# snap-research/3dgp

Measured on AMD Instinct MI355X. Metric: generator-forward img/s @256^2, 64 steps, higher is better.
Workload: dtype f32; 1 GPU; BASELINE configs[2]: ImageNet 256x256, 64(+64) ray steps, cmax 512, c_dim 1000, tri-plane 512^2 x 96, full HIP path; batch_per_gpu=16, global_batch=16, img_resolution=256, num_ray_steps=64, depth_adaptor=False, parallelism=dp1 (batch-sharded, weights replicated)

## Files before the change

3dgp_amd/csrc/sampling.hip:

```cpp
#include "common.h"

namespace {

constexpr int MAXS = 256;
constexpr int RAYS_PER_BLOCK = 4;
constexpr int MAXS_PASS = 512;
constexpr int MAXS_LONG = 1024;

template <int MS>
struct alignas(16) WaveScratchT {
    float z[MS];
    float sig[MS];
    float w[MS + 4];
    float cdf[MS];
    float bins[MS];
    float col[3][MS];
};
using WaveScratch = WaveScratchT<MAXS>;

template <int MS> struct alignas(16) MarchScratchT { float z[MS]; float sig[MS]; float w[MS + 4]; };
template <> struct alignas(16) MarchScratchT<MAXS> : WaveScratch {};
template <int MS> struct alignas(16) UnifyScratchT { float z[MS]; };
template <> struct alignas(16) UnifyScratchT<MAXS> : WaveScratch {};

__device__ __forceinline__ void wave_sync() {
    __builtin_amdgcn_fence(__ATOMIC_ACQ_REL, "wavefront");
    __builtin_amdgcn_wave_barrier();
}

__device__ __forceinline__ float s2t(float s, float t_near, float t_far) { return s * t_far + (1.0f - s) * t_near; }

template <bool LONGX>
__device__ __forceinline__ float exp_neg(float x) { return LONGX ? (float)exp(-(double)x) : expf(-x); }

#define TDGP_CLASSICAL_ALPHA(LONGX, z, sig, i, S, flags, cut_thr, alpha, fac)                                        \
    do {                                                                                                            \
        alpha = 0.f; fac = 1.0f;                                                                                    \
        if ((i) < (S)) {                                                                                            \
            const float delta = ((i) < (S) - 1) ? (z[(i) + 1] - z[i]) : (((flags) & 1) ? 1e10f : 1e-3f);            \
            float sp = ((flags) & 8) ? (sig[i] > 0.f ? sig[i] : 0.f) : softplus20f(sig[i]);                         \
            if (sp < cut_thr) sp = 0.f;              \
            alpha = 1.0f - exp_neg<LONGX>(delta * sp);                                                              \
            fac = (1.0f - alpha) + 1e-10f;                                                                          \
        }                                                                                                           \
    } while (0)

#define TDGP_MIP_ALPHA(LONGX, z, sig, i, S, M, density_bias, cut_thr, alpha, fac)                                    \
    do {                                                                                                            \
        alpha = 0.f; fac = 1.0f;                                                                                    \
        if ((i) < (M)) {                                                                                            \
            float delta, smid;                                                                                      \
            if ((i) < (S) - 1) { delta = z[(i) + 1] - z[i]; smid = (sig[i] + sig[(i) + 1]) / 2.f; }                 \
            else { delta = 1e10f; smid = sig[(S) - 1]; }                                                            \
            float sp = softplus20f(smid + density_bias);                                                            \
            if (sp < cut_thr) sp = 0.f;                                                \
            float dd = sp * delta;                                                                                  \
            alpha = 1.0f - exp_neg<LONGX>(dd);                                                                      \
            fac = (1.0f - alpha) + 1e-10f;                                                                          \
        }                                                                                                           \
    } while (0)

#define TDGP_MARCH_PASS(wi, incl64, alpha, fac, carry)                   \
    const double incl64 = wave_scan_f64<true>((double)(fac)) * (carry);  \
    const float incl = (float)incl64;                                    \
    const float excl = wave_shr1_f32(incl, (float)(carry));              \
    const float wi = (alpha) * excl;
#define TDGP_MARCH_PASS2(wi0, wi1, i1, alpha, fac)                                                                          \
    const double s0 = wave_scan_f64<true>((double)fac[0]), s1 = wave_scan_f64<true>((double)fac[1]);                        \
    const double c1 = wave_last_f64(s0);                                                                                    \
    const double i1 = s1 * c1;                                                                                              \
    const float incl0 = (float)s0, incl1 = (float)i1;                                                                       \
    const float wi0 = alpha[0] * wave_shr1_f32(incl0, 1.0f), wi1 = alpha[1] * wave_shr1_f32(incl1, (float)c1);

template <bool LONGX = false>
__device__ void march_classical_lds(const float* z, const float* sig, float* w, int S, int flags, float cut_thr, float& final_T, float& wagg) {
    const int l = lane_id();
    double carry = 1.0;
    float wsum = 0.0f;
    if (S > 64 && S <= 128) {
        float alpha[2], fac[2];
#pragma unroll
        for (int c = 0; c < 2; c++) {
            const int i = 64 * c + l;
            TDGP_CLASSICAL_ALPHA(LONGX, z, sig, i, S, flags, cut_thr, alpha[c], fac[c]);
        }
        TDGP_MARCH_PASS2(wi0, wi1, i1, alpha, fac)
        w[l] = wi0; wsum += wi0;
        if (64 + l < S) { w[64 + l] = wi1; wsum += wi1; }
        carry = wave_last_f64(i1);
    } else
    for (int base = 0; base < S; base += 64) {
        const int i = base + l;
        float alpha, fac;
        TDGP_CLASSICAL_ALPHA(LONGX, z, sig, i, S, flags, cut_thr, alpha, fac);
        TDGP_MARCH_PASS(wi, incl64, alpha, fac, carry)
        if (i < S) { w[i] = wi; wsum += wi; }
        carry = wave_last_f64(incl64);
    }
    wagg = wave_sum_f32(wsum);
    final_T = (float)carry;
    wave_sync();
    if ((flags & 2) && l == 0) w[S - 1] += (1.0f - wagg);
    wave_sync();
}

template <bool LONGX = false>
__device__ void march_mip_lds(const float* z, const float* sig, float* w, int S, int flags, float density_bias, float cut_thr, float& final_T,
                              float& wagg) {
    const int l = lane_id();
    const int M = (flags & 1) ? S : S - 1;
    double carry = 1.0;
    float wsum = 0.0f;
    for (int base = 0; base < M; base += 64) {
        const int i = base + l;
        float alpha, fac;
        TDGP_MIP_ALPHA(LONGX, z, sig, i, S, M, density_bias, cut_thr, alpha, fac);
        TDGP_MARCH_PASS(wi, incl64, alpha, fac, carry)
        if (i < M) { w[i] = wi; wsum += wi; }
        carry = wave_last_f64(incl64);
    }
    wagg = wave_sum_f32(wsum);
    final_T = (float)carry;
    wave_sync();
}

__device__ float torch_order_sum_lds(const float* w1, int n, float eps) {
    const int l = lane_id();
    if (n >= 8) {
        const int nv = n >> 3, nilp = nv >> 2;
        const int col = l & 7, a = (l >> 3) & 3;
        float acc = 0.f;
        for (int i = 0; i < nilp; i++) acc = __fadd_rn(acc, __fadd_rn(w1[(4 * i + a) * 8 + col], eps));
        for (int j = 4 * nilp; j < nv; j++) {
            const float v = __fadd_rn(w1[j * 8 + col], eps);
            if (a == 0) acc = __fadd_rn(acc, v);
        }
        float p = __shfl(acc, col, 64);
        p = __fadd_rn(p, __shfl(acc, col + 8, 64));
        p = __fadd_rn(p, __shfl(acc, col + 16, 64));
        p = __fadd_rn(p, __shfl(acc, col + 24, 64));
        float fin = 0.f;
        for (int k = nv * 8; k < n; k++) fin = __fadd_rn(fin, __fadd_rn(w1[k], eps));
#pragma unroll
        for (int c = 0; c < 8; c++) fin = __fadd_rn(fin, __int_as_float(__builtin_amdgcn_readlane(__float_as_int(p), c)));
        return fin;
    }
    float acc[4] = {0.f, 0.f, 0.f, 0.f};
    const int nilp = n >> 2;
    if (nilp)
        for (int k = 0; k < 4; k++) acc[k] = __fadd_rn(acc[k], __fadd_rn(w1[k], eps));
    for (int r = 4 * nilp; r < n; r++) acc[0] = __fadd_rn(acc[0], __fadd_rn(w1[r], eps));
    for (int k = 1; k < 4; k++) acc[0] = __fadd_rn(acc[0], acc[k]);
    return acc[0];
}

__device__ __forceinline__ float torch_order_sum_62(const float* w1, int n, float eps) {
    const int l = lane_id();
    const int col = l & 7, a = (l >> 3) & 3;
    float acc = 0.f;
    acc = __fadd_rn(acc, __fadd_rn(w1[a * 8 + col], eps));
#pragma unroll
    for (int j = 4; j < 7; j++) {
        const float v = __fadd_rn(w1[j * 8 + col], eps);
        if (a == 0) acc = __fadd_rn(acc, v);
    }
    float p = __shfl(acc, col, 64);
    p = __fadd_rn(p, __shfl(acc, col + 8, 64));
    p = __fadd_rn(p, __shfl(acc, col + 16, 64));
    p = __fadd_rn(p, __shfl(acc, col + 24, 64));
    float fin = 0.f;
#pragma unroll
    for (int k = 56; k < 62; k++) {
        const float t = __fadd_rn(fin, __fadd_rn(w1[k], eps));
        fin = k < n ? t : fin;
    }
#pragma unroll
    for (int c = 0; c < 8; c++) fin = __fadd_rn(fin, __int_as_float(__builtin_amdgcn_readlane(__float_as_int(p), c)));
    return fin;
}

template <int NV>
__device__ __forceinline__ void smooth_read(const float* w, int Wn, float (&nv)[NV]) {
    const int l = lane_id();
#pragma unroll
    for (int c = 0; c < NV; c++) {
        const int i = l + 64 * c;
        if (i < Wn) {
            float a = (i - 1 >= 0) ? w[i - 1] : -INFINITY, b = w[i], d = (i + 1 < Wn) ? w[i + 1] : -INFINITY;
            float t0 = a > b ? a : b;
            float t1 = b > d ? b : d;
            nv[c] = (t0 + t1) / 2.f + 0.01f;
        }
    }
}
template <int NV>
__device__ __forceinline__ void smooth_write(float* w, int Wn, const float (&nv)[NV]) {
    const int l = lane_id();
#pragma unroll
    for (int c = 0; c < NV; c++) {
        const int i = l + 64 * c;
        if (i < Wn) w[i] = nv[c];
    }
}
__device__ __forceinline__ void offset_weights(float* w, int Wn) {
    for (int i = lane_id(); i < Wn; i += 64) w[i] = w[i] + 1e-5f;
}
template <bool ROW62>
__device__ __forceinline__ void pdf_cdf(const float* z, const float* w, float* bins, float* cdf, int S, int Wn) {
    const int l = lane_id();
    const float eps = 1e-5f;
    const int nb = S - 1, ns = Wn - 2;
    for (int i = l; i < nb; i += 64) bins[i] = 0.5f * (z[i] + z[i + 1]);
    const float totf = ROW62 ? torch_order_sum_62(w + 1, ns, eps) : torch_order_sum_lds(w + 1, ns, eps);
    double carry = 0.0;
    if (l == 0) cdf[0] = 0.f;
    for (int base = 0; base < ns; base += 64) {
        const int i = base + l;
        float pdf = (i < ns) ? (w[1 + i] + eps) / totf : 0.f;
        double incl = wave_scan_f64<false>((double)pdf) + carry;
        if (i < ns) cdf[i + 1] = (float)incl;
        carry = wave_last_f64(incl);
    }
}
__device__ __forceinline__ int cdf_search(const float* cdf, int nc, float uu) {
    int lo = 0, hi = nc;
    while (lo < hi) {
        int mid = (lo + hi) >> 1;
        if (cdf[mid] <= uu) lo = mid + 1; else hi = mid;
    }
    return lo;
}
__device__ __forceinline__ float cdf_sample(const float* cdf, const float* bins, int nb, int ns, int ind, float uu, int& below, int& above) {
    const float eps = 1e-5f;
    below = ind - 1 < 0 ? 0 : ind - 1;
    above = ind > ns ? ns : ind;
    const float cb = cdf[below], ca = cdf[above];
    const float bb = bins[below < nb ? below : nb - 1], ba = bins[above < nb ? above : nb - 1];
    float denom = ca - cb;
    if (denom < eps) denom = 1.f;
    return bb + (uu - cb) / denom * (ba - bb);
}

template <typename SC, typename GetU, typename Emit>
__device__ void importance_lds(SC& sc, int S, int Wn, GetU getu, int N, int mip, Emit emit) {
    const int l = lane_id();
    float* w = sc.w;
    constexpr int CAP = sizeof(sc.z) / sizeof(float), NV = (CAP > MAXS ? CAP : MAXS) / 64;
    if (mip) {
        float nv[NV];
        smooth_read<NV>(w, Wn, nv);
        wave_sync();
        smooth_write<NV>(w, Wn, nv);
    } else {
        offset_weights(w, Wn);
    }
    wave_sync();
    const int nb = S - 1, ns = Wn - 2, nc = ns + 1;
    pdf_cdf<false>(sc.z, w, sc.bins, sc.cdf, S, Wn);
    wave_sync();
    for (int j = l; j < N; j += 64) {
        const float uu = getu(j);
        const int ind = cdf_search(sc.cdf, nc, uu);
        int below, above;
        const float smp = cdf_sample(sc.cdf, sc.bins, nb, ns, ind, uu, below, above);
        emit(j, smp, ind, below, above);
    }
}

__device__ __forceinline__ float strat_one(float u, int k, int S, float step, int marcher) {
    auto lin = [&](int q) { return (S == 1) ? 0.f : ((q < S / 2) ? __fmaf_rn(step, (float)q, 0.f) : __fmaf_rn(-step, (float)(S - 1 - q), 1.f)); };
    if (marcher == 0) {
        const float lower = (k == 0) ? lin(0) : 0.5f * (lin(k) + lin(k - 1));
        const float upper = (k == S - 1) ? lin(S - 1) : 0.5f * (lin(k + 1) + lin(k));
        return lower + (upper - lower) * u;
    }
    const float delta = (float)((1.0 - 0.0) / (double)(S - 1));
    return lin(k) + u * delta;
}

__global__ __launch_bounds__(256) void stratified_kernel(const float* __restrict__ u, float* __restrict__ sdist, float* __restrict__ tdist,
                                                        int64_t n, int S, int marcher, float t_near, float t_far) {
    const float step = (1.f - 0.f) / (float)(S - 1);
    for (int64_t i = blockIdx.x * (int64_t)blockDim.x + threadIdx.x; i < n; i += (int64_t)gridDim.x * blockDim.x) {
        const float s = strat_one(u[i], (int)(i % S), S, step, marcher);
        sdist[i] = s;
        if (tdist) tdist[i] = s2t(s, t_near, t_far);
    }
}

__global__ __launch_bounds__(256) void stratified4_kernel(const float4* __restrict__ u, float4* __restrict__ sdist, float4* __restrict__ tdist,
                                                         int64_t n4, int S, int marcher, float t_near, float t_far) {
    const float step = (1.f - 0.f) / (float)(S - 1);
    const int S4 = S >> 2;
    for (int64_t i = blockIdx.x * (int64_t)blockDim.x + threadIdx.x; i < n4; i += (int64_t)gridDim.x * blockDim.x) {
        const int k = (int)(i % S4) * 4;
        const float4 uu = u[i];
        const float4 s = make_float4(strat_one(uu.x, k, S, step, marcher), strat_one(uu.y, k + 1, S, step, marcher), strat_one(uu.z, k + 2, S, step, marcher),
                                     strat_one(uu.w, k + 3, S, step, marcher));
        sdist[i] = s;
        if (tdist) tdist[i] = make_float4(s2t(s.x, t_near, t_far), s2t(s.y, t_near, t_far), s2t(s.z, t_near, t_far), s2t(s.w, t_near, t_far));
    }
}

__global__ __launch_bounds__(256) void density_activation_kernel(const float* __restrict__ x, float* __restrict__ y, int64_t n, int relu, float bias) {
    for (int64_t i = blockIdx.x * (int64_t)blockDim.x + threadIdx.x; i < n; i += (int64_t)gridDim.x * blockDim.x)
        y[i] = relu ? (x[i] > 0.f ? x[i] : 0.f) : softplus20f(x[i] + bias);
}

template <int MS>
__global__ __launch_bounds__(256) void ray_march_kernel(const float* __restrict__ colors, const float* __restrict__ dens,
                                                       const float* __restrict__ depths, float* __restrict__ rgb, float* __restrict__ depth_o,
                                                       float* __restrict__ weights, float* __restrict__ final_T, int64_t rays, int S, int C,
                                                       int marcher, int flags, float density_bias, float cut_thr) {
    __shared__ MarchScratchT<MS> scratch[RAYS_PER_BLOCK];
    const int wv = threadIdx.x >> 6, l = lane_id();
    const int64_t r = (int64_t)blockIdx.x * RAYS_PER_BLOCK + wv;
    if (r >= rays) return;
    MarchScratchT<MS>& sc = scratch[wv];
    for (int i = l; i < S; i += 64) { sc.z[i] = depths[r * S + i]; sc.sig[i] = dens[r * S + i]; }
    wave_sync();
    float fT, wagg;
    const int M = (marcher == 0) ? S : ((flags & 1) ? S : S - 1);
    if (MS > MAXS && S > MAXS) {
        if (marcher == 0) march_classical_lds<(MS > MAXS)>(sc.z, sc.sig, sc.w, S, flags, cut_thr, fT, wagg);
        else march_mip_lds<(MS > MAXS)>(sc.z, sc.sig, sc.w, S, flags, density_bias, cut_thr, fT, wagg);
    } else
    if (marcher == 0) march_classical_lds(sc.z, sc.sig, sc.w, S, flags, cut_thr, fT, wagg);
    else march_mip_lds(sc.z, sc.sig, sc.w, S, flags, density_bias, cut_thr, fT, wagg);
    if (weights) for (int i = l; i < M; i += 64) weights[r * M + i] = sc.w[i];
    for (int c = 0; c <= C; c++) {
        float acc = 0.0f;
        for (int i = l; i < M; i += 64) {
            float v;
            if (c < C) {
                v = colors[(r * S + i) * C + c];
                if (marcher == 1 && i < S - 1) v = (v + colors[(r * S + i + 1) * C + c]) / 2.f;
            } else {
                v = sc.z[i];
                if (marcher == 1 && i < S - 1) v = (v + sc.z[i + 1]) / 2.f;
            }
            acc += sc.w[i] * v;
        }
        float out = wave_sum_f32(acc);
        if (marcher == 1 && c < C) {
            if (flags & 4) out = out + 1.0f - wagg;
            out = out * 2.0f - 1.0f;
        }
        if (l == 0) { if (c < C) rgb[r * C + c] = out; else depth_o[r] = out; }
    }
    if (l == 0) final_T[r] = fT;
}

template <int MS>
__global__ __launch_bounds__(256) void sample_importance_kernel(const float* __restrict__ z, const float* __restrict__ weights,
                                                               const float* __restrict__ u, float* __restrict__ samples, int32_t* __restrict__ inds,
                                                               int32_t* __restrict__ below, int32_t* __restrict__ above, float* __restrict__ cdf_o,
                                                               int64_t rays, int S, int Wn, int N, int mip) {
    __shared__ WaveScratchT<MS> scratch[RAYS_PER_BLOCK];
    const int wv = threadIdx.x >> 6, l = lane_id();
    const int64_t r = (int64_t)blockIdx.x * RAYS_PER_BLOCK + wv;
    if (r >= rays) return;
    WaveScratchT<MS>& sc = scratch[wv];
    for (int i = l; i < S; i += 64) sc.z[i] = z[r * S + i];
    for (int i = l; i < Wn; i += 64) sc.w[i] = weights[r * Wn + i];
    wave_sync();
    importance_lds(sc, S, Wn, [&](int j) { return u[r * N + j]; }, N, mip, [&](int j, float smp, int ind, int bl, int ab) {
        samples[r * N + j] = smp;
        if (inds) { inds[r * N + j] = ind; below[r * N + j] = bl; above[r * N + j] = ab; }
    });
    if (cdf_o) for (int i = l; i < Wn - 1; i += 64) cdf_o[r * (Wn - 1) + i] = sc.cdf[i];
}

template <int NS>
__device__ __forceinline__ void stable_ranks_n(const float* key, int M, int* rank) {
    const int l = lane_id();
    float k[NS];
#pragma unroll
    for (int c = 0; c < NS; c++) { const int i = l + 64 * c; k[c] = i < M ? key[i] : 0.f; rank[c] = 0; }
#pragma unroll 4
    for (int m = 0; m < M; m++) {
        const float km = key[m];
#pragma unroll
        for (int c = 0; c < NS; c++) {
            const int i = l + 64 * c;
            rank[c] += (km < k[c] || (km == k[c] && m < i)) ? 1 : 0;
        }
    }
}
template <int NR>
__device__ __forceinline__ void stable_ranks(const float* key, int M, int (&rank)[NR]) {
    static_assert(NR == MAXS / 64 || NR == MAXS_PASS / 64 || NR == MAXS_LONG / 64, "stable_ranks: 4, 8 or 16 slots");
#pragma unroll
    for (int c = 0; c < NR; c++) rank[c] = 0;
    if constexpr (NR == MAXS / 64) {
        if (M <= 64) stable_ranks_n<1>(key, M, rank);
        else if (M <= 128) stable_ranks_n<2>(key, M, rank);
        else if (M <= 192) stable_ranks_n<3>(key, M, rank);
        else stable_ranks_n<4>(key, M, rank);
    } else {
        if (M <= MAXS_PASS) stable_ranks_n<MAXS_PASS / 64>(key, M, rank);
        else stable_ranks_n<NR>(key, M, rank);
    }
}

template <int NS, int CAP>
__device__ __forceinline__ void wave_bitonic_sort_n(float (&key)[CAP], int (&idx)[CAP]) {
    static_assert(NS <= CAP && (NS & (NS - 1)) == 0, "wave_bitonic_sort_n: NS a power of two within the arrays");
    const int l = lane_id();
#pragma unroll
    for (int k = 2; k <= 64 * NS; k <<= 1) {
#pragma unroll
        for (int j = k >> 1; j > 0; j >>= 1) {
            if (j >= 64) {
                const int js = j >> 6;
#pragma unroll
                for (int c = 0; c < NS; c++) {
                    if (c & js) continue;
                    const int c2 = c | js;
                    const bool asc = ((64 * c) & k) == 0;
                    const bool less2 = key[c2] < key[c] || (key[c2] == key[c] && idx[c2] < idx[c]);
                    if (less2 == asc) { const float tk = key[c]; key[c] = key[c2]; key[c2] = tk; const int ti = idx[c]; idx[c] = idx[c2]; idx[c2] = ti; }
                }
            } else {
#pragma unroll
                for (int c = 0; c < NS; c++) {
                    const float pk = __shfl_xor(key[c], j, 64);
                    const int pi = __shfl_xor(idx[c], j, 64);
                    const bool asc = ((64 * c + l) & k) == 0;
                    const bool keep_min = ((l & j) == 0) == asc;
                    const bool partner_less = pk < key[c] || (pk == key[c] && pi < idx[c]);
                    if (partner_less == keep_min) { key[c] = pk; idx[c] = pi; }
                }
            }
        }
    }
}

template <int MS>
__global__ __launch_bounds__(256) void importance_from_coarse_kernel(const float* __restrict__ rgbs, const float* __restrict__ sdist,
                                                                    const float* __restrict__ u_fine, float* __restrict__ tfine,
                                                                    float* __restrict__ sfine, int32_t* __restrict__ inds,
                                                                    int32_t* __restrict__ fine_perm, int64_t rays, int S, int N,
                                                                    int marcher, int flags, float density_bias, float cut_thr, float t_near, float t_far) {
    __shared__ WaveScratchT<MS> scratch[RAYS_PER_BLOCK];
    const int wv = threadIdx.x >> 6, l = lane_id();
    const int64_t r = (int64_t)blockIdx.x * RAYS_PER_BLOCK + wv;
    if (r >= rays) return;
    WaveScratchT<MS>& sc = scratch[wv];
    for (int i = l; i < S; i += 64) { sc.z[i] = sdist[r * S + i]; sc.sig[i] = rgbs[(r * S + i) * 4 + 3]; }
    float upre[MS / 64];
    if constexpr (MS > MAXS) {
        for (int i = l; i < N; i += 64) sc.col[1][i] = u_fine[r * N + i];
    } else {
#pragma unroll
    for (int c = 0; c < MS / 64; c++) upre[c] = (l + 64 * c < N) ? u_fine[r * N + l + 64 * c] : 0.f;
    }
    wave_sync();
    float fT, wagg;
    int Wn = S;
    if (MS > MAXS && S > MAXS) {
        if (marcher == 0) march_classical_lds<(MS > MAXS)>(sc.z, sc.sig, sc.w, S, flags, cut_thr, fT, wagg);
        else { march_mip_lds<(MS > MAXS)>(sc.z, sc.sig, sc.w, S, flags, density_bias, cut_thr, fT, wagg); Wn = (flags & 1) ? S : S - 1; }
    } else
    if (marcher == 0) march_classical_lds(sc.z, sc.sig, sc.w, S, flags, cut_thr, fT, wagg);
    else { march_mip_lds(sc.z, sc.sig, sc.w, S, flags, density_bias, cut_thr, fT, wagg); Wn = (flags & 1) ? S : S - 1; }
    float* tkey = sc.col[0];
    if constexpr (MS > MAXS)
        [[clang::always_inline]] importance_lds(sc, S, Wn, [&](int j) { return sc.col[1][j]; }, N, marcher, [&](int j, float smp, int ind, int, int) {
            tkey[j] = s2t(smp, t_near, t_far);
            if (sfine) sfine[r * N + j] = smp;
            if (inds) inds[r * N + j] = ind;
        });
    else
    importance_lds(sc, S, Wn, [&](int j) { float v = upre[0];
#pragma unroll
                                          for (int c = 1; c < MS / 64; c++) v = (j >> 6) == c ? upre[c] : v;
                                          return v; }, N, marcher, [&](int j, float smp, int ind, int, int) {
        tkey[j] = s2t(smp, t_near, t_far);
        if (sfine) sfine[r * N + j] = smp;
        if (inds) inds[r * N + j] = ind;
    });
    wave_sync();
    if (N <= 64) {
        float key = l < N ? tkey[l] : INFINITY;
        {
            if (l >= N) tkey[l] = INFINITY;
            wave_sync();
            int cnt = 0;
#pragma unroll
            for (int jj = 0; jj < 16; jj++) {
                const float4 k4 = *(const float4*)&tkey[4 * jj];
                cnt += (k4.x < key ? 1 : 0) + (k4.y < key ? 1 : 0) + (k4.z < key ? 1 : 0) + (k4.w < key ? 1 : 0);
            }
            int* slot = (int*)sc.bins;
            if (l < N) slot[cnt] = l;
            wave_sync();
            const bool mine = l >= N || slot[cnt] == l;
            if (__all(mine)) {
                if (l < N) {
                    const int src = slot[l];
                    tfine[r * N + l] = tkey[src];
                    if (fine_perm) fine_perm[r * N + l] = src;
                }
                return;
            }
        }
        float k1[1] = {key};
        int idx[1] = {l};
        wave_bitonic_sort_n<1>(k1, idx);
        if (l < N) {
            tfine[r * N + l] = k1[0];
            if (fine_perm) fine_perm[r * N + l] = idx[0];
        }
        return;
    }
    if (N <= 128) {
        float key[2] = {tkey[l], l + 64 < N ? tkey[l + 64] : INFINITY};
        {
            if (l + 64 >= N) tkey[l + 64] = INFINITY;
            wave_sync();
            int cnt[2] = {0, 0};
#pragma unroll 8
            for (int jj = 0; jj < 32; jj++) {
                const float4 k4 = *(const float4*)&tkey[4 * jj];
#pragma unroll
                for (int c = 0; c < 2; c++)
                    cnt[c] += (k4.x < key[c] ? 1 : 0) + (k4.y < key[c] ? 1 : 0) + (k4.z < key[c] ? 1 : 0) + (k4.w < key[c] ? 1 : 0);
            }
            int* slot = (int*)sc.bins;
            slot[cnt[0]] = l;
            if (l + 64 < N) slot[cnt[1]] = l + 64;
            wave_sync();
            const bool mine = slot[cnt[0]] == l && (l + 64 >= N || slot[cnt[1]] == l + 64);
            if (__all(mine)) {
#pragma unroll
                for (int c = 0; c < 2; c++) {
                    const int pos = l + 64 * c;
                    if (pos < N) {
                        const int src = slot[pos];
                        tfine[r * N + pos] = tkey[src];
                        if (fine_perm) fine_perm[r * N + pos] = src;
                    }
                }
                return;
            }
        }
        int idx[2] = {l, l + 64};
        wave_bitonic_sort_n<2>(key, idx);
#pragma unroll
        for (int c = 0; c < 2; c++) {
            const int pos = l + 64 * c;
            if (pos < N) {
                tfine[r * N + pos] = key[c];
                if (fine_perm) fine_perm[r * N + pos] = idx[c];
            }
        }
        return;
    }
    if constexpr (MS > MAXS) {
        constexpr int NSL = MS / 64;
        float key[NSL];
        int idx[NSL];
#pragma unroll
        for (int c = 0; c < NSL; c++) { const int e = l + 64 * c; key[c] = e < N ? tkey[e] : INFINITY; idx[c] = e; }
        if (N <= 256) wave_bitonic_sort_n<4>(key, idx);
        else wave_bitonic_sort_n<NSL>(key, idx);
#pragma unroll
        for (int c = 0; c < NSL; c++) {
            const int pos = l + 64 * c;
            if (pos < N) {
                tfine[r * N + pos] = key[c];
                if (fine_perm) fine_perm[r * N + pos] = idx[c];
            }
        }
        return;
    } else {
    int rank[MAXS / 64];
    stable_ranks(tkey, N, rank);
#pragma unroll
    for (int c = 0; c < MAXS / 64; c++) {
        const int j = l + 64 * c;
        if (j < N) {
            tfine[r * N + rank[c]] = tkey[j];
            if (fine_perm) fine_perm[r * N + rank[c]] = j;
        }
    }
    }
}

template <int MS>
__global__ __launch_bounds__(256) void unify_kernel(const float* __restrict__ d1, const float* __restrict__ c1, const float* __restrict__ s1, int S1,
                                                   const float* __restrict__ d2, const float* __restrict__ c2, const float* __restrict__ s2, int S2,
                                                   float* __restrict__ d, float* __restrict__ c, float* __restrict__ s, int32_t* __restrict__ perm,
                                                   int64_t rays, int C) {
    __shared__ UnifyScratchT<MS> scratch[RAYS_PER_BLOCK];
    const int wv = threadIdx.x >> 6, l = lane_id();
    const int64_t r = (int64_t)blockIdx.x * RAYS_PER_BLOCK + wv;
    if (r >= rays) return;
    UnifyScratchT<MS>& sc = scratch[wv];
    const int M = S1 + S2;
    for (int i = l; i < M; i += 64) sc.z[i] = i < S1 ? d1[r * S1 + i] : d2[r * S2 + (i - S1)];
    wave_sync();
    int rank[MS / 64];
    stable_ranks(sc.z, M, rank);
#pragma unroll
    for (int cc = 0; cc < MS / 64; cc++) {
        const int i = l + 64 * cc;
        if (i >= M) continue;
        const int pos = rank[cc];
        d[r * M + pos] = sc.z[i];
        s[r * M + pos] = i < S1 ? s1[r * S1 + i] : s2[r * S2 + (i - S1)];
        for (int k = 0; k < C; k++) c[(r * M + pos) * C + k] = i < S1 ? c1[(r * S1 + i) * C + k] : c2[(r * S2 + (i - S1)) * C + k];
        if (perm) perm[r * M + pos] = i;
    }
}

template <int MS>
__global__ __launch_bounds__(256) void merge_composite_kernel(const float* __restrict__ rgbs1, const float* __restrict__ t1, int S1,
                                                             const float* __restrict__ rgbs2, const float* __restrict__ t2, int S2,
                                                             float* __restrict__ rgb, float* __restrict__ depth_o, float* __restrict__ wsum_o,
                                                             float* __restrict__ final_T, int32_t* __restrict__ perm, const int32_t* __restrict__ perm2, int64_t rays,
                                                             int marcher, int flags, float density_bias, float cut_thr) {
    __shared__ WaveScratchT<MS> scratch[RAYS_PER_BLOCK];
    const int wv = threadIdx.x >> 6, l = lane_id();
    const int64_t r = (int64_t)blockIdx.x * RAYS_PER_BLOCK + wv;
    if (r >= rays) return;
    WaveScratchT<MS>& sc = scratch[wv];
    const int M = S1 + S2;
    float4 cval[MS / 64];
#pragma unroll
    for (int cc = 0; cc < MS / 64; cc++) {
        const int i = l + 64 * cc;
        if (i < M) {
            sc.cdf[i] = i < S1 ? t1[r * S1 + i] : t2[r * S2 + (i - S1)];
            cval[cc] = i < S1 ? ((const float4*)rgbs1)[r * S1 + i] : ((const float4*)rgbs2)[r * S2 + (i - S1)];
        }
    }
    wave_sync();
    bool bad = false;
    for (int i = l; i < M; i += 64)
        if (i + 1 < M && i + 1 != S1 && sc.cdf[i + 1] < sc.cdf[i]) bad = true;
    constexpr int RK = (MS > MAXS ? MS : MAXS) / 64;
    int rank[RK];
    if (__any(bad)) {
        stable_ranks(sc.cdf, M, rank);
    } else {
        constexpr int NSL = MS / 64;
        float v[NSL];
        int lo[NSL], hi[NSL];
        bool fine[NSL];
        int* const last = (int*)sc.bins;
        for (int c = l; c <= S1 && c < MS; c += 64) last[c] = 0;
#pragma unroll
        for (int cc = 0; cc < NSL; cc++) {
            const int i = l + 64 * cc;
            v[cc] = i < M ? sc.cdf[i] : 0.f;
            fine[cc] = i >= S1 && i < M;
            lo[cc] = 0;
            hi[cc] = fine[cc] ? S1 : 0;
        }
        const int steps = 32 - __clz(S1);
        for (int it = 0; it < steps; it++) {
#pragma unroll
            for (int cc = 0; cc < NSL; cc++) {
                if (64 * cc + 64 <= S1) continue;
                const bool open = lo[cc] < hi[cc];
                const int mid = (lo[cc] + hi[cc]) >> 1;
                const float o = sc.cdf[open ? mid : 0];
                const bool right = o <= v[cc];
                lo[cc] = (open && right) ? mid + 1 : lo[cc];
                hi[cc] = (open && !right) ? mid : hi[cc];
            }
        }
        wave_sync();
#pragma unroll
        for (int cc = 0; cc < NSL; cc++) {
            const int i = l + 64 * cc;
            if (fine[cc]) atomicMax(&last[lo[cc]], i - S1 + 1);
        }
        wave_sync();
#pragma unroll
        for (int cc = 0; cc < RK; cc++) rank[cc] = 0;
        int carry = 0;
#pragma unroll
        for (int cc = 0; cc < NSL; cc++) {
            const int i = l + 64 * cc;
            if (64 * cc < S1) {
                const int incl = max(wave_scan_max_i32((i <= S1 && i < MS) ? last[i] : 0), carry);
                carry = wave_last_i32(incl);
                rank[cc] = fine[cc] ? (i - S1) + lo[cc] : i + incl;
            } else {
                rank[cc] = (i - S1) + lo[cc];
            }
        }
    }
#pragma unroll
    for (int cc = 0; cc < MS / 64; cc++) {
        const int i = l + 64 * cc;
        if (i >= M) continue;
        const int pos = rank[cc];
        const float4 v = cval[cc];
        sc.z[pos] = sc.cdf[i];
        sc.col[0][pos] = v.x; sc.col[1][pos] = v.y; sc.col[2][pos] = v.z; sc.sig[pos] = v.w;
        if (perm) perm[r * M + pos] = i < S1 ? i : S1 + (perm2 ? perm2[r * S2 + (i - S1)] : i - S1);
    }
    wave_sync();
    float fT, wagg;
    const int Mm = (marcher == 0) ? M : ((flags & 1) ? M : M - 1);
    if (MS > MAXS && M > MAXS) {
        if (marcher == 0) march_classical_lds<(MS > MAXS)>(sc.z, sc.sig, sc.w, M, flags, cut_thr, fT, wagg);
        else march_mip_lds<(MS > MAXS)>(sc.z, sc.sig, sc.w, M, flags, density_bias, cut_thr, fT, wagg);
    } else
    if (marcher == 0) march_classical_lds(sc.z, sc.sig, sc.w, M, flags, cut_thr, fT, wagg);
    else march_mip_lds(sc.z, sc.sig, sc.w, M, flags, density_bias, cut_thr, fT, wagg);
    float acc[4] = {0.f, 0.f, 0.f, 0.f}, wacc = 0.f;
    for (int i = l; i < Mm; i += 64) {
        const float wi = sc.w[i];
        wacc += wi;
#pragma unroll
        for (int c = 0; c < 4; c++) {
            float v = c < 3 ? sc.col[c][i] : sc.z[i];
            if (marcher == 1 && i < M - 1) v = (v + (c < 3 ? sc.col[c][i + 1] : sc.z[i + 1])) / 2.f;
            acc[c] += wi * v;
        }
    }
    float out[4];
#pragma unroll
    for (int c = 0; c < 4; c++) out[c] = wave_sum_f32(acc[c]);
    const float wtot = wave_sum_f32(wacc);
    if (marcher == 1) {
#pragma unroll
        for (int c = 0; c < 3; c++) {
            if (flags & 4) out[c] = out[c] + 1.0f - wagg;
            out[c] = out[c] * 2.0f - 1.0f;
        }
    }
    if (l == 0) {
        rgb[r * 3 + 0] = out[0]; rgb[r * 3 + 1] = out[1]; rgb[r * 3 + 2] = out[2];
        depth_o[r] = out[3];
        if (wsum_o) wsum_o[r] = wtot;
        if (final_T) final_T[r] = fT;
    }
}

constexpr int PAIR_RAYS_PER_BLOCK = 8;

struct alignas(16) ImpPairScratch { float z[64]; float sig[64]; float w[64 + 4]; float cdf[64]; float bins[64]; float key[64]; };

struct ImpRay {
    ImpPairScratch* sc;
    int64_t r;
    bool live;
    float zl, sg, u;
    float nv[1];
    float key[1];
    int cnt, idx[1];
};

__device__ __forceinline__ void imp_load(ImpRay& R, const float* __restrict__ rgbs, const float* __restrict__ sdist, const float* __restrict__ u_fine) {
    const int l = lane_id();
    R.zl = sdist[R.r * 64 + l]; R.sg = rgbs[(R.r * 64 + l) * 4 + 3]; R.u = u_fine[R.r * 64 + l];
}
__device__ __forceinline__ void imp_park(ImpRay& R) { const int l = lane_id(); R.sc->z[l] = R.zl; R.sc->sig[l] = R.sg; }
__device__ __forceinline__ float imp_march(ImpRay& R, int marcher, int flags, float density_bias, float cut_thr) {
    const int l = lane_id();
    const int M = (marcher == 0 || (flags & 1)) ? 64 : 63;
    float alpha, fac;
    const float *z = R.sc->z, *sig = R.sc->sig;
    if (marcher == 0) { TDGP_CLASSICAL_ALPHA(false, z, sig, l, 64, flags, cut_thr, alpha, fac); }
    else { TDGP_MIP_ALPHA(false, z, sig, l, 64, M, density_bias, cut_thr, alpha, fac); }
    const double carry = 1.0;
    TDGP_MARCH_PASS(wi, incl64, alpha, fac, carry)
    float wsum = 0.0f;
    if (l < M) { R.sc->w[l] = wi; wsum += wi; }
    return wave_sum_f32(wsum);
}
__device__ __forceinline__ void imp_last_back(ImpRay& R, float wagg) { if (lane_id() == 0) R.sc->w[63] += (1.0f - wagg); }
__device__ __forceinline__ void imp_search(ImpRay& R, int Wn, float t_near, float t_far, float* __restrict__ sfine, int32_t* __restrict__ inds) {
    const int l = lane_id();
    ImpPairScratch& sc = *R.sc;
    const int ns = Wn - 2, nc = ns + 1;
    const float uu = R.u;
    const int ind = cdf_search(sc.cdf, nc, uu);
    int below, above;
    const float smp = cdf_sample(sc.cdf, sc.bins, 63, ns, ind, uu, below, above);
    R.key[0] = s2t(smp, t_near, t_far);
    sc.key[l] = R.key[0];
    if (R.live) {
        if (sfine) sfine[R.r * 64 + l] = smp;
        if (inds) inds[R.r * 64 + l] = ind;
    }
}
__device__ __forceinline__ void imp_count(ImpRay& R) {
    const int l = lane_id();
    int cnt = 0;
#pragma unroll
    for (int jj = 0; jj < 16; jj++) {
        const float4 k4 = *(const float4*)&R.sc->key[4 * jj];
        cnt += (k4.x < R.key[0] ? 1 : 0) + (k4.y < R.key[0] ? 1 : 0) + (k4.z < R.key[0] ? 1 : 0) + (k4.w < R.key[0] ? 1 : 0);
    }
    R.cnt = cnt;
    ((int*)R.sc->bins)[cnt] = l;
}
__device__ __forceinline__ bool imp_gather(ImpRay& R) {
    const int l = lane_id();
    const int* slot = (const int*)R.sc->bins;
    const bool ok = __all(slot[R.cnt] == l);
    const int src = ok ? slot[l] : l;
    R.key[0] = R.sc->key[src];
    R.idx[0] = src;
    return ok;
}
__device__ __forceinline__ void imp_store(const ImpRay& R, float* __restrict__ tfine, int32_t* __restrict__ fine_perm) {
    const int l = lane_id();
    if (R.live) {
        tfine[R.r * 64 + l] = R.key[0];
        if (fine_perm) fine_perm[R.r * 64 + l] = R.idx[0];
    }
}

__global__ __launch_bounds__(256, 8) void importance_from_coarse_pair_kernel(const float* __restrict__ rgbs, const float* __restrict__ sdist,
                                                                            const float* __restrict__ u_fine, float* __restrict__ tfine,
                                                                            float* __restrict__ sfine, int32_t* __restrict__ inds,
                                                                            int32_t* __restrict__ fine_perm, int64_t rays, int marcher, int flags,
                                                                            float density_bias, float cut_thr, float t_near, float t_far) {
    __shared__ ImpPairScratch scratch[PAIR_RAYS_PER_BLOCK];
    const int wv = threadIdx.x >> 6;
    const int64_t r0 = ((int64_t)blockIdx.x * (PAIR_RAYS_PER_BLOCK / 2) + wv) * 2;
    if (r0 >= rays) return;
    ImpRay A, B;
    A.sc = &scratch[2 * wv]; A.r = r0; A.live = true;
    B.sc = &scratch[2 * wv + 1]; B.live = r0 + 1 < rays; B.r = B.live ? r0 + 1 : r0;
    imp_load(A, rgbs, sdist, u_fine); imp_load(B, rgbs, sdist, u_fine);
    imp_park(A); imp_park(B);
    wave_sync();
    const float waA = imp_march(A, marcher, flags, density_bias, cut_thr), waB = imp_march(B, marcher, flags, density_bias, cut_thr);
    wave_sync();
    int Wn = 64;
    if (marcher == 0) {
        if (flags & 2) { imp_last_back(A, waA); imp_last_back(B, waB); }
        wave_sync();
        offset_weights(A.sc->w, Wn); offset_weights(B.sc->w, Wn);
    } else {
        Wn = (flags & 1) ? 64 : 63;
        smooth_read<1>(A.sc->w, Wn, A.nv); smooth_read<1>(B.sc->w, Wn, B.nv);
        wave_sync();
        smooth_write<1>(A.sc->w, Wn, A.nv); smooth_write<1>(B.sc->w, Wn, B.nv);
    }
    wave_sync();
    pdf_cdf<true>(A.sc->z, A.sc->w, A.sc->bins, A.sc->cdf, 64, Wn); pdf_cdf<true>(B.sc->z, B.sc->w, B.sc->bins, B.sc->cdf, 64, Wn);
    wave_sync();
    imp_search(A, Wn, t_near, t_far, sfine, inds); imp_search(B, Wn, t_near, t_far, sfine, inds);
    wave_sync();
    imp_count(A); imp_count(B);
    wave_sync();
    const bool okA = imp_gather(A), okB = imp_gather(B);
    if (!okA) wave_bitonic_sort_n<1>(A.key, A.idx);
    if (!okB) wave_bitonic_sort_n<1>(B.key, B.idx);
    imp_store(A, tfine, fine_perm); imp_store(B, tfine, fine_perm);
}

struct alignas(16) MergePairScratch {
    float key[128];
    float z[128];
    float sig[128];
    float col[3][128];
};

struct MergeRay {
    MergePairScratch* sc;
    int64_t r;
    bool live;
    float k[2];
    float4 c[2];
    int p2;
    int lo;
    int rank[2];
    bool bad;
};

__device__ __forceinline__ void mrg_load(MergeRay& R, const float* __restrict__ rgbs1, const float* __restrict__ t1, const float* __restrict__ rgbs2,
                                         const float* __restrict__ t2, const int32_t* __restrict__ perm2, bool want_perm) {
    const int l = lane_id();
    R.k[0] = t1[R.r * 64 + l]; R.k[1] = t2[R.r * 64 + l];
    R.c[0] = ((const float4*)rgbs1)[R.r * 64 + l]; R.c[1] = ((const float4*)rgbs2)[R.r * 64 + l];
    R.p2 = (want_perm && perm2) ? perm2[R.r * 64 + l] : l;
}
__device__ __forceinline__ void mrg_park(MergeRay& R) { const int l = lane_id(); R.sc->key[l] = R.k[0]; R.sc->key[64 + l] = R.k[1]; }
__device__ __forceinline__ void mrg_search(MergeRay& R) {
    const int l = lane_id();
    const float* key = R.sc->key;
    R.bad = l < 63 && (key[l + 1] < key[l] || key[64 + l + 1] < key[64 + l]);
    int* const last = (int*)R.sc->z;
    last[l] = 0;
    if (l == 0) last[64] = 0;
    const float v = R.k[1];
    int lo = 0, hi = 64;
#pragma unroll
    for (int it = 0; it < 7; it++) {
        const bool open = lo < hi;
        const int mid = (lo + hi) >> 1;
        const bool right = key[open ? mid : 0] <= v;
        lo = (open && right) ? mid + 1 : lo;
        hi = (open && !right) ? mid : hi;
    }
    R.lo = lo;
}
__device__ __forceinline__ void mrg_scatter_last(MergeRay& R) { atomicMax(&((int*)R.sc->z)[R.lo], lane_id() + 1); }
__device__ __forceinline__ bool mrg_ranks(MergeRay& R) {
    const int l = lane_id();
    const int incl = max(wave_scan_max_i32(((const int*)R.sc->z)[l]), 0);
    R.rank[0] = l + incl;
    R.rank[1] = l + R.lo;
    return __any(R.bad);
}
__device__ __forceinline__ void mrg_scatter(MergeRay& R, int32_t* __restrict__ perm) {
    const int l = lane_id();
    MergePairScratch& sc = *R.sc;
#pragma unroll
    for (int cc = 0; cc < 2; cc++) {
        const int pos = R.rank[cc];
        const float4 v = R.c[cc];
        sc.z[pos] = R.k[cc];
        sc.col[0][pos] = v.x; sc.col[1][pos] = v.y; sc.col[2][pos] = v.z; sc.sig[pos] = v.w;
        if (perm && R.live) perm[R.r * 128 + pos] = cc == 0 ? l : 64 + R.p2;
    }
}
__device__ __forceinline__ void mrg_march(MergeRay& R, int marcher, int flags, float density_bias, float cut_thr, float& final_T, float& wagg) {
    const int l = lane_id();
    MergePairScratch& sc = *R.sc;
    float* w = sc.key;
    double carry = 1.0;
    float wsum = 0.0f;
    if (marcher == 0) {
        float alpha[2], fac[2];
#pragma unroll
        for (int c = 0; c < 2; c++) { const int i = 64 * c + l; TDGP_CLASSICAL_ALPHA(false, sc.z, sc.sig, i, 128, flags, cut_thr, alpha[c], fac[c]); }
        TDGP_MARCH_PASS2(wi0, wi1, i1, alpha, fac)
        w[l] = wi0; wsum += wi0;
        w[64 + l] = wi1; wsum += wi1;
        carry = wave_last_f64(i1);
    } else {
        const int M = (flags & 1) ? 128 : 127;
#pragma unroll
        for (int base = 0; base < 128; base += 64) {
            const int i = base + l;
            float alpha, fac;
            TDGP_MIP_ALPHA(false, sc.z, sc.sig, i, 128, M, density_bias, cut_thr, alpha, fac);
            TDGP_MARCH_PASS(wi, incl64, alpha, fac, carry)
            if (i < M) { w[i] = wi; wsum += wi; }
            carry = wave_last_f64(incl64);
        }
    }
    wagg = wave_sum_f32(wsum);
    final_T = (float)carry;
}
__device__ __forceinline__ void mrg_last_back(MergeRay& R, float wagg) { if (lane_id() == 0) R.sc->key[127] += (1.0f - wagg); }
__device__ __forceinline__ void mrg_composite(MergeRay& R, int marcher, int flags, float wagg, float fT, float* __restrict__ rgb, float* __restrict__ depth_o,
                                              float* __restrict__ wsum_o, float* __restrict__ final_T) {
    const int l = lane_id();
    const MergePairScratch& sc = *R.sc;
    const float* w = sc.key;
    const int Mm = (marcher == 0 || (flags & 1)) ? 128 : 127;
    float acc[4] = {0.f, 0.f, 0.f, 0.f}, wacc = 0.f;
#pragma unroll
    for (int i = l; i < 128; i += 64) {
        if (i < Mm) {
            const float wi = w[i];
            wacc += wi;
#pragma unroll
            for (int c = 0; c < 4; c++) {
                float v = c < 3 ? sc.col[c][i] : sc.z[i];
                if (marcher == 1 && i < 127) v = (v + (c < 3 ? sc.col[c][i + 1] : sc.z[i + 1])) / 2.f;
                acc[c] += wi * v;
            }
        }
    }
    float out[4];
#pragma unroll
    for (int c = 0; c < 4; c++) out[c] = wave_sum_f32(acc[c]);
    const float wtot = wave_sum_f32(wacc);
    if (marcher == 1) {
#pragma unroll
        for (int c = 0; c < 3; c++) {
            if (flags & 4) out[c] = out[c] + 1.0f - wagg;
            out[c] = out[c] * 2.0f - 1.0f;
        }
    }
    if (l == 0 && R.live) {
        rgb[R.r * 3 + 0] = out[0]; rgb[R.r * 3 + 1] = out[1]; rgb[R.r * 3 + 2] = out[2];
        depth_o[R.r] = out[3];
        if (wsum_o) wsum_o[R.r] = wtot;
        if (final_T) final_T[R.r] = fT;
    }
}

__global__ __launch_bounds__(256, 8) void merge_composite_pair_kernel(const float* __restrict__ rgbs1, const float* __restrict__ t1,
                                                                     const float* __restrict__ rgbs2, const float* __restrict__ t2,
                                                                     float* __restrict__ rgb, float* __restrict__ depth_o, float* __restrict__ wsum_o,
                                                                     float* __restrict__ final_T, int32_t* __restrict__ perm, const int32_t* __restrict__ perm2,
                                                                     int64_t rays, int marcher, int flags, float density_bias, float cut_thr) {
    __shared__ MergePairScratch scratch[PAIR_RAYS_PER_BLOCK];
    const int wv = threadIdx.x >> 6;
    const int64_t r0 = ((int64_t)blockIdx.x * (PAIR_RAYS_PER_BLOCK / 2) + wv) * 2;
    if (r0 >= rays) return;
    MergeRay A, B;
    A.sc = &scratch[2 * wv]; A.r = r0; A.live = true;
    B.sc = &scratch[2 * wv + 1]; B.live = r0 + 1 < rays; B.r = B.live ? r0 + 1 : r0;
    mrg_load(A, rgbs1, t1, rgbs2, t2, perm2, perm != nullptr); mrg_load(B, rgbs1, t1, rgbs2, t2, perm2, perm != nullptr);
    mrg_park(A); mrg_park(B);
    wave_sync();
    mrg_search(A); mrg_search(B);
    wave_sync();
    mrg_scatter_last(A); mrg_scatter_last(B);
    wave_sync();
    const bool slowA = mrg_ranks(A), slowB = mrg_ranks(B);
    if (slowA) stable_ranks_n<2>(A.sc->key, 128, A.rank);
    if (slowB) stable_ranks_n<2>(B.sc->key, 128, B.rank);
    wave_sync();
    mrg_scatter(A, perm); mrg_scatter(B, perm);
    wave_sync();
    float fTA, waA, fTB, waB;
    mrg_march(A, marcher, flags, density_bias, cut_thr, fTA, waA); mrg_march(B, marcher, flags, density_bias, cut_thr, fTB, waB);
    wave_sync();
    if (marcher == 0 && (flags & 2)) { mrg_last_back(A, waA); mrg_last_back(B, waB); }
    wave_sync();
    mrg_composite(A, marcher, flags, waA, fTA, rgb, depth_o, wsum_o, final_T); mrg_composite(B, marcher, flags, waB, fTB, rgb, depth_o, wsum_o, final_T);
}

#define TDGP_LAUNCH_RAYS(NAME, KERNEL, PER_BLOCK, ...)                                                                                   \
    do {                                                                                                                                 \
        TDGP_LAUNCH(NAME, KERNEL, dim3((int)cdiv64(rays, PER_BLOCK)), dim3(256), 0, (hipStream_t)stream, __VA_ARGS__);                   \
        TDGP_LAUNCH_CHECK();                                                                                                             \
    } while (0)

}

TDGP_API int tdgp_sample_stratified(const float* u, float* sdist, float* tdist, int64_t rays, int S, int marcher, float t_near,
                                    float t_far, tdgp_stream_t stream) {
    TDGP_CHECK(u && sdist, TDGP_EINVAL, "sample_stratified: null pointer");
    TDGP_CHECK(S >= 2 && rays >= 0, TDGP_EINVAL, "sample_stratified: need S >= 2");
    TDGP_CHECK(marcher == 0 || marcher == 1, TDGP_EINVAL, "sample_stratified: unknown ray marcher %d", marcher);
    const int64_t n = rays * S;
    if (n == 0) return TDGP_OK;
    if ((S & 3) == 0 && (((uintptr_t)u | (uintptr_t)sdist | (uintptr_t)tdist) & 15) == 0) {
        TDGP_LAUNCH("stratified_kernel", stratified4_kernel, dim3((int)min((int64_t)8192, cdiv64(n / 4, 256))), dim3(256), 0, (hipStream_t)stream, (const float4*)u,
                    (float4*)sdist, (float4*)tdist, n / 4, S, marcher, t_near, t_far);
        TDGP_LAUNCH_CHECK();
        return TDGP_OK;
    }
    TDGP_LAUNCH("stratified_kernel", stratified_kernel, dim3((int)min((int64_t)8192, cdiv64(n, 256))), dim3(256), 0, (hipStream_t)stream, u, sdist, tdist, n, S,
                       marcher, t_near, t_far);
    TDGP_LAUNCH_CHECK();
    return TDGP_OK;
}

TDGP_API int tdgp_density_activation(const float* sigma, float* out, int64_t n, int flags, float density_bias, tdgp_stream_t stream) {
    TDGP_CHECK(sigma && out, TDGP_EINVAL, "density_activation: null pointer");
    TDGP_CHECK(n >= 0, TDGP_EINVAL, "density_activation: negative length");
    if (n == 0) return TDGP_OK;
    TDGP_LAUNCH("density_activation_kernel", density_activation_kernel, dim3((int)min((int64_t)8192, cdiv64(n, 256))), dim3(256), 0, (hipStream_t)stream, sigma, out, n,
                (flags & 8) ? 1 : 0, density_bias);
    TDGP_LAUNCH_CHECK();
    return TDGP_OK;
}

TDGP_API int tdgp_ray_march(const float* colors, const float* densities, const float* depths, float* rgb, float* depth, float* weights,
                            float* final_T, int64_t rays, int S, int C, int marcher, int flags, float density_bias, float cut_threshold, tdgp_stream_t stream) {
    TDGP_CHECK(colors && densities && depths && rgb && depth && final_T, TDGP_EINVAL, "ray_march: null pointer");
    TDGP_CHECK(S >= 2 && S <= MAXS_LONG, TDGP_EUNSUPPORTED, "ray_march: S=%d outside [2,%d] (a merged list of at most %d + %d samples)", S, MAXS_LONG,
               MAXS_PASS, MAXS_PASS);
    TDGP_CHECK(C >= 1 && C <= 8, TDGP_EUNSUPPORTED, "ray_march: C=%d outside [1,8]", C);
    TDGP_CHECK(marcher == 0 || marcher == 1, TDGP_EINVAL, "ray_march: unknown ray marcher %d", marcher);
    TDGP_FAULT_CHECK("ray_march");
    if (rays == 0) return TDGP_OK;
    TDGP_LAUNCH_RAYS("ray_march_kernel", S <= MAXS ? ray_march_kernel<MAXS> : ray_march_kernel<MAXS_LONG>, RAYS_PER_BLOCK, colors, densities, depths, rgb, depth,
                     weights, final_T, rays, S, C, marcher, flags, density_bias, cut_threshold);
    return TDGP_OK;
}

TDGP_API int tdgp_sample_importance(const float* z, const float* weights, const float* u, float* samples, int32_t* inds, int32_t* below,
                                    int32_t* above, float* cdf, int64_t rays, int S, int Wn, int N, int marcher, tdgp_stream_t stream) {
    TDGP_CHECK(z && weights && u && samples, TDGP_EINVAL, "sample_importance: null pointer");
    TDGP_CHECK(!inds || (below && above), TDGP_EINVAL, "sample_importance: inds/below/above come together");
    TDGP_CHECK(S >= 4 && S <= MAXS_PASS && Wn >= 3 && Wn <= S && N >= 1, TDGP_EUNSUPPORTED,
               "sample_importance: bad S=%d Wn=%d N=%d (S at most %d: beyond it torch's sum order is not restated)", S, Wn, N, MAXS_PASS);
    if (rays == 0) return TDGP_OK;
    TDGP_LAUNCH_RAYS("sample_importance_kernel", S <= MAXS ? sample_importance_kernel<MAXS> : sample_importance_kernel<MAXS_PASS>, RAYS_PER_BLOCK, z, weights, u,
                     samples, inds, below, above, cdf, rays, S, Wn, N, marcher);
    return TDGP_OK;
}

TDGP_API int tdgp_unify_samples(const float* d1, const float* c1, const float* s1, int S1, const float* d2, const float* c2, const float* s2,
                                int S2, float* d, float* c, float* s, int32_t* perm, int64_t rays, int C, tdgp_stream_t stream) {
    TDGP_CHECK(d1 && c1 && s1 && d2 && c2 && s2 && d && c && s, TDGP_EINVAL, "unify_samples: null pointer");
    TDGP_CHECK(S1 >= 1 && S2 >= 1 && S1 + S2 <= MAXS_LONG, TDGP_EUNSUPPORTED, "unify_samples: S1+S2=%d > %d", S1 + S2, MAXS_LONG);
    if (rays == 0) return TDGP_OK;
    TDGP_LAUNCH_RAYS("unify_kernel", S1 + S2 <= MAXS ? unify_kernel<MAXS> : unify_kernel<MAXS_LONG>, RAYS_PER_BLOCK, d1, c1, s1, S1, d2, c2, s2, S2, d, c, s, perm,
                     rays, C);
    return TDGP_OK;
}

TDGP_API int tdgp_importance_from_coarse(const float* rgbs_coarse, const float* sdist, const float* u_fine, float* tdist_fine,
                                         float* sdist_fine, int32_t* inds, int32_t* fine_perm, int64_t rays, int S, int N, int marcher, int flags,
                                         float density_bias, float cut_threshold, float t_near, float t_far, tdgp_stream_t stream) {
    TDGP_CHECK(rgbs_coarse && sdist && u_fine && tdist_fine, TDGP_EINVAL, "importance_from_coarse: null pointer");
    TDGP_CHECK(S >= 4 && S <= MAXS_PASS && N >= 1 && N <= MAXS_PASS, TDGP_EUNSUPPORTED, "importance_from_coarse: bad S=%d N=%d (both at most %d)", S, N, MAXS_PASS);
    TDGP_CHECK(marcher == 0 || marcher == 1, TDGP_EINVAL, "importance_from_coarse: unknown ray marcher %d", marcher);
    TDGP_FAULT_CHECK("importance_from_coarse");
    if (rays == 0) return TDGP_OK;
    if (S == 64 && N == 64) {
        TDGP_LAUNCH_RAYS("importance_from_coarse_kernel", importance_from_coarse_pair_kernel, PAIR_RAYS_PER_BLOCK, rgbs_coarse, sdist, u_fine, tdist_fine, sdist_fine,
                         inds, fine_perm, rays, marcher, flags, density_bias, cut_threshold, t_near, t_far);
        return TDGP_OK;
    }
    const bool fits = S <= MAXS && N <= MAXS;
    const auto kernel = (S <= 128 && N <= 128) ? importance_from_coarse_kernel<128> : fits ? importance_from_coarse_kernel<MAXS> : importance_from_coarse_kernel<MAXS_PASS>;
    TDGP_LAUNCH_RAYS("importance_from_coarse_kernel", kernel, RAYS_PER_BLOCK, rgbs_coarse, sdist, u_fine, tdist_fine, sdist_fine, inds, fine_perm, rays, S, N, marcher,
                     flags, density_bias, cut_threshold, t_near, t_far);
    return TDGP_OK;
}

TDGP_API int tdgp_merge_composite(const float* rgbs_coarse, const float* t_coarse, int S1, const float* rgbs_fine, const float* t_fine, int S2,
                                  float* rgb, float* depth, float* wsum, float* final_T, int32_t* perm, const int32_t* fine_perm, int64_t rays,
                                  int marcher, int flags, float density_bias, float cut_threshold, tdgp_stream_t stream) {
    TDGP_CHECK(rgbs_coarse && t_coarse && rgbs_fine && t_fine && rgb && depth, TDGP_EINVAL, "merge_composite: null pointer");
    TDGP_CHECK(S1 >= 1 && S2 >= 1 && S1 + S2 <= MAXS_LONG, TDGP_EUNSUPPORTED, "merge_composite: S1+S2=%d > %d", S1 + S2, MAXS_LONG);
    TDGP_CHECK(marcher == 0 || marcher == 1, TDGP_EINVAL, "merge_composite: unknown ray marcher %d", marcher);
    TDGP_FAULT_CHECK("merge_composite");
    if (rays == 0) return TDGP_OK;
    if (S1 == 64 && S2 == 64) {
        TDGP_LAUNCH_RAYS("merge_composite_kernel", merge_composite_pair_kernel, PAIR_RAYS_PER_BLOCK, rgbs_coarse, t_coarse, rgbs_fine, t_fine, rgb, depth, wsum, final_T,
                         perm, fine_perm, rays, marcher, flags, density_bias, cut_threshold);
        return TDGP_OK;
    }
    const int M = S1 + S2;
    const auto kernel = M <= 128 ? merge_composite_kernel<128> : M <= 192 ? merge_composite_kernel<192> : M <= MAXS ? merge_composite_kernel<MAXS>
                      : M <= MAXS_PASS ? merge_composite_kernel<MAXS_PASS> : merge_composite_kernel<MAXS_LONG>;
    TDGP_LAUNCH_RAYS("merge_composite_kernel", kernel, RAYS_PER_BLOCK, rgbs_coarse, t_coarse, S1, rgbs_fine, t_fine, S2, rgb, depth, wsum, final_T, perm, fine_perm,
                     rays, marcher, flags, density_bias, cut_threshold);
    return TDGP_OK;
}
```

Measured before the change: 723.2 img/s.

## Replace binary searches with two-level counting and precompute sort ranks from uniforms

Replaces the serial binary searches over the CDF in importance sampling and over keys in the merge kernel with a two-level count. The count reads an 8-entry top index of segment maxima, then one 8-wide segment, using float4 LDS reads. The importance kernel also computes the sort permutation early from the uniform draws, since sampled positions are monotone in u, and overlaps it with marching. A monotonicity check falls back to bitonic sort, and fewer wave syncs are needed. The cost is extra LDS writes for the top index and NaN padding of the CDF row, plus reuse of the sig scratch buffer, which risks aliasing.

```diff
diff --git a/3dgp_amd/csrc/sampling.hip b/3dgp_amd/csrc/sampling.hip
--- a/3dgp_amd/csrc/sampling.hip
+++ b/3dgp_amd/csrc/sampling.hip
@@ -206,7 +206,7 @@
     for (int i = lane_id(); i < Wn; i += 64) w[i] = w[i] + 1e-5f;
 }
 template <bool ROW62>
-__device__ __forceinline__ void pdf_cdf(const float* z, const float* w, float* bins, float* cdf, int S, int Wn) {
+__device__ __forceinline__ void pdf_cdf(const float* z, const float* w, float* bins, float* cdf, int S, int Wn, float* top = nullptr) {
     const int l = lane_id();
     const float eps = 1e-5f;
     const int nb = S - 1, ns = Wn - 2;
@@ -219,8 +219,22 @@
         float pdf = (i < ns) ? (w[1 + i] + eps) / totf : 0.f;
         double incl = wave_scan_f64<false>((double)pdf) + carry;
         if (i < ns) cdf[i + 1] = (float)incl;
+        if constexpr (ROW62) {
+            const float knot = i < ns ? (float)incl : __builtin_nanf("");
+            if (i >= ns && i < 63) cdf[i + 1] = knot;
+            if ((l & 7) == 6) top[l >> 3] = knot;
+        }
         carry = wave_last_f64(incl);
     }
+}
+__device__ __forceinline__ int count_le8(const float* p, float v) {
+    const float4 a = *(const float4*)p, b = *(const float4*)(p + 4);
+    return (a.x <= v ? 1 : 0) + (a.y <= v ? 1 : 0) + (a.z <= v ? 1 : 0) + (a.w <= v ? 1 : 0) + (b.x <= v ? 1 : 0) + (b.y <= v ? 1 : 0) + (b.z <= v ? 1 : 0) +
+           (b.w <= v ? 1 : 0);
+}
+__device__ __forceinline__ int two_level_count(const float* row, const float* top, float v) {
+    const int seg = min(count_le8(top, v), 7);
+    return 8 * seg + count_le8(row + 8 * seg, v);
 }
 __device__ __forceinline__ int cdf_search(const float* cdf, int nc, float uu) {
     int lo = 0, hi = nc;
@@ -755,13 +769,15 @@
     float nv[1];
     float key[1];
     int cnt, idx[1];
+    int src;
+    bool ok;
 };
 
 __device__ __forceinline__ void imp_load(ImpRay& R, const float* __restrict__ rgbs, const float* __restrict__ sdist, const float* __restrict__ u_fine) {
     const int l = lane_id();
     R.zl = sdist[R.r * 64 + l]; R.sg = rgbs[(R.r * 64 + l) * 4 + 3]; R.u = u_fine[R.r * 64 + l];
 }
-__device__ __forceinline__ void imp_park(ImpRay& R) { const int l = lane_id(); R.sc->z[l] = R.zl; R.sc->sig[l] = R.sg; }
+__device__ __forceinline__ void imp_park(ImpRay& R) { const int l = lane_id(); R.sc->z[l] = R.zl; R.sc->sig[l] = R.sg; R.sc->key[l] = R.u; R.key[0] = R.u; }
 __device__ __forceinline__ float imp_march(ImpRay& R, int marcher, int flags, float density_bias, float cut_thr) {
     const int l = lane_id();
     const int M = (marcher == 0 || (flags & 1)) ? 64 : 63;
@@ -779,9 +795,9 @@
 __device__ __forceinline__ void imp_search(ImpRay& R, int Wn, float t_near, float t_far, float* __restrict__ sfine, int32_t* __restrict__ inds) {
     const int l = lane_id();
     ImpPairScratch& sc = *R.sc;
-    const int ns = Wn - 2, nc = ns + 1;
+    const int ns = Wn - 2;
     const float uu = R.u;
-    const int ind = cdf_search(sc.cdf, nc, uu);
+    const int ind = two_level_count(sc.cdf, sc.sig, uu);
     int below, above;
     const float smp = cdf_sample(sc.cdf, sc.bins, 63, ns, ind, uu, below, above);
     R.key[0] = s2t(smp, t_near, t_far);
@@ -802,14 +818,19 @@
     R.cnt = cnt;
     ((int*)R.sc->bins)[cnt] = l;
 }
-__device__ __forceinline__ bool imp_gather(ImpRay& R) {
+__device__ __forceinline__ void imp_slot(ImpRay& R) {
     const int l = lane_id();
     const int* slot = (const int*)R.sc->bins;
-    const bool ok = __all(slot[R.cnt] == l);
-    const int src = ok ? slot[l] : l;
-    R.key[0] = R.sc->key[src];
-    R.idx[0] = src;
-    return ok;
+    R.ok = __all(slot[R.cnt] == l);
+    R.src = R.ok ? slot[l] : l;
+}
+__device__ __forceinline__ bool imp_take(ImpRay& R) {
+    const int l = lane_id();
+    const float k = R.sc->key[R.src];
+    const bool good = R.ok && __all(wave_shr1_f32(k, -INFINITY) < k);
+    if (good) R.key[0] = k;
+    R.idx[0] = good ? R.src : l;
+    return good;
 }
 __device__ __forceinline__ void imp_store(const ImpRay& R, float* __restrict__ tfine, int32_t* __restrict__ fine_perm) {
     const int l = lane_id();
@@ -835,26 +856,25 @@
     imp_park(A); imp_park(B);
     wave_sync();
     const float waA = imp_march(A, marcher, flags, density_bias, cut_thr), waB = imp_march(B, marcher, flags, density_bias, cut_thr);
+    imp_count(A); imp_count(B);
     wave_sync();
     int Wn = 64;
     if (marcher == 0) {
         if (flags & 2) { imp_last_back(A, waA); imp_last_back(B, waB); }
-        wave_sync();
-        offset_weights(A.sc->w, Wn); offset_weights(B.sc->w, Wn);
     } else {
         Wn = (flags & 1) ? 64 : 63;
         smooth_read<1>(A.sc->w, Wn, A.nv); smooth_read<1>(B.sc->w, Wn, B.nv);
-        wave_sync();
-        smooth_write<1>(A.sc->w, Wn, A.nv); smooth_write<1>(B.sc->w, Wn, B.nv);
-    }
-    wave_sync();
-    pdf_cdf<true>(A.sc->z, A.sc->w, A.sc->bins, A.sc->cdf, 64, Wn); pdf_cdf<true>(B.sc->z, B.sc->w, B.sc->bins, B.sc->cdf, 64, Wn);
+    }
+    imp_slot(A); imp_slot(B);
+    wave_sync();
+    if (marcher == 0) { offset_weights(A.sc->w, Wn); offset_weights(B.sc->w, Wn); }
+    else { smooth_write<1>(A.sc->w, Wn, A.nv); smooth_write<1>(B.sc->w, Wn, B.nv); }
+    wave_sync();
+    pdf_cdf<true>(A.sc->z, A.sc->w, A.sc->bins, A.sc->cdf, 64, Wn, A.sc->sig); pdf_cdf<true>(B.sc->z, B.sc->w, B.sc->bins, B.sc->cdf, 64, Wn, B.sc->sig);
     wave_sync();
     imp_search(A, Wn, t_near, t_far, sfine, inds); imp_search(B, Wn, t_near, t_far, sfine, inds);
     wave_sync();
-    imp_count(A); imp_count(B);
-    wave_sync();
-    const bool okA = imp_gather(A), okB = imp_gather(B);
+    const bool okA = imp_take(A), okB = imp_take(B);
     if (!okA) wave_bitonic_sort_n<1>(A.key, A.idx);
     if (!okB) wave_bitonic_sort_n<1>(B.key, B.idx);
     imp_store(A, tfine, fine_perm); imp_store(B, tfine, fine_perm);
@@ -886,7 +906,11 @@
     R.c[0] = ((const float4*)rgbs1)[R.r * 64 + l]; R.c[1] = ((const float4*)rgbs2)[R.r * 64 + l];
     R.p2 = (want_perm && perm2) ? perm2[R.r * 64 + l] : l;
 }
-__device__ __forceinline__ void mrg_park(MergeRay& R) { const int l = lane_id(); R.sc->key[l] = R.k[0]; R.sc->key[64 + l] = R.k[1]; }
+__device__ __forceinline__ void mrg_park(MergeRay& R) {
+    const int l = lane_id();
+    R.sc->key[l] = R.k[0]; R.sc->key[64 + l] = R.k[1];
+    if ((l & 7) == 7) R.sc->sig[l >> 3] = R.k[0];
+}
 __device__ __forceinline__ void mrg_search(MergeRay& R) {
     const int l = lane_id();
     const float* key = R.sc->key;
@@ -894,17 +918,7 @@
     int* const last = (int*)R.sc->z;
     last[l] = 0;
     if (l == 0) last[64] = 0;
-    const float v = R.k[1];
-    int lo = 0, hi = 64;
-#pragma unroll
-    for (int it = 0; it < 7; it++) {
-        const bool open = lo < hi;
-        const int mid = (lo + hi) >> 1;
-        const bool right = key[open ? mid : 0] <= v;
-        lo = (open && right) ? mid + 1 : lo;
-        hi = (open && !right) ? mid : hi;
-    }
-    R.lo = lo;
+    R.lo = two_level_count(key, R.sc->sig, R.k[1]);
 }
 __device__ __forceinline__ void mrg_scatter_last(MergeRay& R) { atomicMax(&((int*)R.sc->z)[R.lo], lane_id() + 1); }
 __device__ __forceinline__ bool mrg_ranks(MergeRay& R) {
```

Result: no change. 724.2 img/s, median of 4 (+0.1%).
